# SimeonZhang/detectron2_tensorflow

Measured on AMD Instinct MI355X. Metric: img/sec whole-node Mask R-CNN R50-FPN @1333x800, higher is better.
Workload: dtype f32

## Files before the change

detectron2_tensorflow_amd/csrc/conv_mfma.hip:

```cpp
#include "common.h"
#include "conv_plan.h"
#include "internal.h"

#include <mutex>
#include <vector>

namespace d2mi {
namespace {

typedef float floatx16 __attribute__((ext_vector_type(16)));

constexpr int BK = kConvBK, LDSP = 36, LDSB = 32;

__device__ __forceinline__ int swz(int row, int elem) {
  return row * LDSB + ((((elem >> 3) ^ (row >> 2)) & 3) << 3) + (elem & 7);
}

typedef short bf16x8 __attribute__((ext_vector_type(8)));

enum EpiFlags {
  kRelu = 1, kReluAfterResidual = 2, kSplit3 = 4, kFlipTaps = 8, kMaskByResidual = 16
};

#ifndef D2MI_CONV_ABLATE
#define D2MI_CONV_ABLATE 0
#endif
constexpr int kAblate = D2MI_CONV_ABLATE;

constexpr bool kPrioMfma = true;

struct ConvArgs {
  const float* x;
  const float* w;
  const float* bias;
  const float* topdown;
  const float* residual;
  const float* gate;
  float* y;
  float* partial;
  int N, H, W, Cin, Cout, KH, KW, stride, pad, OH, OW, flags;
  int M, nM, nN, ntiles, splits, kt_per_split, nk, cchunks;
  int tile_base, m_base, m_end;
  int lds_epi;
  int nt_store;
  int x_bytes, w_bytes;
  int tdH, tdW;
  int reg_partials;
  int xcd2;
  int nlev;
  const float* lv_x[kMaxConvLevels];
  float* lv_y[kMaxConvLevels];
  const float* lv_gate[kMaxConvLevels];
  int lv_H[kMaxConvLevels], lv_W[kMaxConvLevels], lv_OH[kMaxConvLevels], lv_OW[kMaxConvLevels];
  int lv_N[kMaxConvLevels], lv_xbytes[kMaxConvLevels], lv_tile0[kMaxConvLevels + 1];
  int lv_moff[kMaxConvLevels + 1];
  const int32_t* rows;
  const int32_t* nrows;
  int rows_stride;
};

struct Geo {
  const float* x;
  float* y;
  const float* gate;
  int N, H, W, OH, OW, M, m_end, x_bytes;
  int pstride, prow0;
};

__device__ __forceinline__ Geo geo_of(const ConvArgs& a) {
  return Geo{a.x, a.y, a.gate, a.N, a.H, a.W, a.OH, a.OW, a.M, a.m_end, a.x_bytes,
             a.m_end - a.m_base, a.m_base};
}

__device__ __forceinline__ Geo select_level(const ConvArgs& a, int& tile) {
  Geo r = geo_of(a);
  if (a.nlev == 0) return r;
  int base = 0;
#pragma unroll
  for (int l = 0; l < kMaxConvLevels; ++l) {
    if (l < a.nlev && tile >= a.lv_tile0[l]) {
      base = a.lv_tile0[l];
      r.x = a.lv_x[l];
      r.y = a.lv_y[l];
      r.gate = a.lv_gate[l];
      r.N = a.lv_N[l];
      r.H = a.lv_H[l];
      r.W = a.lv_W[l];
      r.OH = a.lv_OH[l];
      r.OW = a.lv_OW[l];
      r.x_bytes = a.lv_xbytes[l];
      r.prow0 = -a.lv_moff[l];
    }
  }
  tile -= base;
  r.M = r.N * r.OH * r.OW;
  r.m_end = r.M;
  r.pstride = a.lv_moff[a.nlev > 0 ? kMaxConvLevels : 0];
  return r;
}

__device__ __forceinline__ float4 ld4(const float* p) { return *reinterpret_cast<const float4*>(p); }
// ... 829 lines not shown
#pragma unroll
      for (int j = 0; j < TN; ++j)
        fb[pb][j] = *reinterpret_cast<const bf16x8*>(
            &B16[pb * BN * LDSB + swz((wc * TN + j) * 32 + li, ks * 16 + lh * 8)]);
    };
    auto mm1 = [&](int pa, int pb) {
      if constexpr ((kAblate & 4) != 0) {
        asm volatile("" ::"v"(fa[pa][0]), "v"(fa[pa][1]), "v"(fb[pb][0]), "v"(fb[pb][1]));
        return;
      }
#pragma unroll
      for (int i = 0; i < TM; ++i)
#pragma unroll
        for (int j = 0; j < TN; ++j)
          acc[i][j] =
              __builtin_amdgcn_mfma_f32_32x32x16_bf16(fa[pa][i], fb[pb][j], acc[i][j], 0, 0, 0);
    };
    auto step16 = [&](int buf, int ks) {
      const uint16_t* A16 = reinterpret_cast<const uint16_t*>(smem + buf * STAGE);
      const uint16_t* B16 = A16 + 3 * BM * LDSB;
      ld1(A16, B16, 1, 1, ks);
      __builtin_amdgcn_sched_barrier(0);
      ld1(A16, B16, 2, 0, ks);
      mm1(1, 1);
      __builtin_amdgcn_sched_barrier(0);
      ld1(A16, B16, 0, 2, ks);
      mm1(2, 0);
      __builtin_amdgcn_sched_barrier(0);
      mm1(0, 2);
      mm1(0, 1);
      mm1(1, 0);
      mm1(0, 0);
    };
    __syncthreads();
    for (int u = 0; u < nks; ++u) {
      const int buf = u & 1;
      if (kPrioMfma) __builtin_amdgcn_s_setprio(1);
      step16(buf, 0);
      step16(buf, 1);
      if (kPrioMfma) __builtin_amdgcn_s_setprio(0);
      __builtin_amdgcn_sched_barrier(0);
      __syncthreads();
    }
  }
  if constexpr ((kAblate & 8) != 0) return;
  if (a.splits > 1 && a.reg_partials) {
    if (wave < 8) store_partial<WN, TM, TN>(a, g, acc, m0, n0, wr, wc, lane, split);
    return;
  }
  store_outputs_lds<WM, WN, TM, TN, 1024>(a, g, acc, m0, n0, wr, wc, lane, split, a.splits > 1,
                                          smem);
}

__global__ void split3_kernel(const float4* __restrict__ x, int64_t n4, uint2* __restrict__ out) {
  for (int64_t i = blockIdx.x * (int64_t)blockDim.x + threadIdx.x; i < n4;
       i += (int64_t)gridDim.x * blockDim.x) {
    uint2 h, m, l;
    split3(x[i], h, m, l);
    out[i] = h;
    out[n4 + i] = m;
    out[2 * n4 + i] = l;
  }
}

__global__ void splitk_reduce_kernel(ConvArgs a) {
  const Geo g = geo_of(a);
  const int64_t total = (int64_t)(a.m_end - a.m_base) * a.Cout;
  for (int64_t i = blockIdx.x * (int64_t)blockDim.x + threadIdx.x; i < total;
       i += (int64_t)gridDim.x * blockDim.x) {
    float acc = 0.f;
#pragma unroll 4
    for (int s = 0; s < a.splits; ++s) acc += a.partial[(size_t)s * total + i];
    const int ml = (int)(i / a.Cout), co = (int)(i - (int64_t)ml * a.Cout);
    const int m = a.m_base + ml;
    a.y[(size_t)m * a.Cout + co] = epilogue(a, g, acc, m, co);
  }
}

__device__ __forceinline__ float4 epilogue4(const ConvArgs& a, const Geo& g, float4 acc, int m,
                                            int co) {
  float4 v = acc;
  if (a.bias) {
    const float4 b = *reinterpret_cast<const float4*>(a.bias + co);
    v = make_float4(v.x + b.x, v.y + b.y, v.z + b.z, v.w + b.w);
  } else {
    v = make_float4(v.x + 0.f, v.y + 0.f, v.z + 0.f, v.w + 0.f);
  }
  const bool relu = (a.flags & kRelu) != 0, after = (a.flags & kReluAfterResidual) != 0;
  if (relu && !after) v = make_float4(fmaxf(v.x, 0.f), fmaxf(v.y, 0.f), fmaxf(v.z, 0.f), fmaxf(v.w, 0.f));
  if (a.topdown) {
    const int n = m / (g.OH * g.OW);
    const int rem = m - n * g.OH * g.OW;
    const int oh = rem / g.OW, ow = rem - oh * g.OW;
    const float4 t = *reinterpret_cast<const float4*>(
        a.topdown + (((size_t)n * a.tdH + (oh >> 1)) * a.tdW + (ow >> 1)) * a.Cout + co);
    v = make_float4(v.x + t.x, v.y + t.y, v.z + t.z, v.w + t.w);
  }
  if (a.residual) {
    const float4 r = *reinterpret_cast<const float4*>(a.residual + (size_t)m * a.Cout + co);
    v = make_float4(v.x + r.x, v.y + r.y, v.z + r.z, v.w + r.w);
  }
  if (relu && after) v = make_float4(fmaxf(v.x, 0.f), fmaxf(v.y, 0.f), fmaxf(v.z, 0.f), fmaxf(v.w, 0.f));
  if (g.gate) {
    const float4 q = *reinterpret_cast<const float4*>(g.gate + (size_t)m * a.Cout + co);
    if (!(q.x > 0.f)) v.x = 0.f;
    if (!(q.y > 0.f)) v.y = 0.f;
// ... 209 lines not shown
  D2MI_REQUIRE(n >= 0 && (n == 0 || (w_hwio && dims && w_packed)), "bad pack table");
  PackMany p = {};
  auto flush = [&]() -> int {
    if (p.n == 0) return 0;
    hipLaunchKernelGGL(pack_weights_many_kernel, dim3(p.block0[p.n]), dim3(256), 0,
                       as_stream(stream), p);
    D2MI_LAUNCH_CHECK();
    p = PackMany{};
    return 0;
  };
  for (int i = 0; i < n; ++i) {
    const int KH = dims[4 * i], KW = dims[4 * i + 1], Cin = dims[4 * i + 2], Cout = dims[4 * i + 3];
    D2MI_REQUIRE(KH > 0 && KW > 0 && Cin > 0 && Cout > 0, "bad conv weight shape (entry %d)", i);
    if (Cin % 64 != 0) {
      const int rc = d2mi_conv_pack_weights(w_hwio[i], KH, KW, Cin, Cout, w_packed[i], stream);
      if (rc) return rc;
      continue;
    }
    const long long blocks = (long long)KH * KW * ((Cout + 63) / 64) * (Cin / 64);
    if (p.n == kMaxPack || (long long)p.block0[p.n] + blocks > (1LL << 30)) {
      const int rc = flush();
      if (rc) return rc;
    }
    p.w[p.n] = w_hwio[i];
    p.out[p.n] = w_packed[i];
    p.Cin[p.n] = Cin;
    p.Cout[p.n] = Cout;
    p.block0[p.n + 1] = p.block0[p.n] + (int)blocks;
    ++p.n;
  }
  return flush();
}

extern "C" int d2mi_conv_pack_weights(const float* w_hwio, int KH, int KW, int Cin, int Cout,
                                      float* w_packed, void* stream) {
  D2MI_REQUIRE(KH > 0 && KW > 0 && Cin > 0 && Cout > 0, "bad conv weight shape");
  if (Cin % 64 == 0) {
    hipLaunchKernelGGL(pack_weights_tiled_kernel, dim3((Cout + 63) / 64, Cin / 64, KH * KW),
                       dim3(256), 0, as_stream(stream), w_hwio, Cin, Cout, w_packed);
    D2MI_LAUNCH_CHECK();
    return 0;
  }
  const int64_t total = (int64_t)KH * KW * Cin * Cout;
  const int grid = (int)std::min<int64_t>((total + 255) / 256, 8192);
  hipLaunchKernelGGL(pack_weights_kernel, dim3(grid), dim3(256), 0, as_stream(stream), w_hwio,
                     KH * KW, Cin, Cout, w_packed);
  D2MI_LAUNCH_CHECK();
  return 0;
}

template <bool SPLIT, bool ML>
static void launch_conv(int family, dim3 grid, hipStream_t st, const ConvArgs& a) {
  if (family == kConvWS256x128) {
    if constexpr (SPLIT && !ML) hipLaunchKernelGGL((conv_ws_kernel<2>), grid, dim3(1024), 0, st, a);
  } else if (family == kConv128x128) {
    hipLaunchKernelGGL((conv_mfma_kernel<2, 2, 2, 2, false, SPLIT, 3, ML>), grid, dim3(256), 0, st,
                       a);
  } else if (family == kConv128x64) {
    hipLaunchKernelGGL((conv_mfma_kernel<4, 1, 1, 2, true, SPLIT, 2, ML>), grid, dim3(256), 0, st,
                       a);
  } else {
    hipLaunchKernelGGL((conv_mfma_kernel<4, 1, 1, 1, true, SPLIT, 2, ML>), grid, dim3(256), 0, st,
                       a);
  }
}

template <int TN, int KMAX>
static void launch_stream1x1_t(const ConvPlan& p, hipStream_t st, const ConvArgs& a) {
  const int nt = tuning(kTuneConvStreamNt);
  constexpr int W = 8;
  const dim3 grid(p.grid);
  if (p.form == 3) {
    if constexpr (TN == 2)
      hipLaunchKernelGGL((conv1x1_stream_kernel<TN, KMAX, W, true, true>), grid, dim3(64 * W), 0,
                         st, a, p.nslices, nt);
  } else if (p.form == 1) {
    hipLaunchKernelGGL((conv1x1_stream_kernel<TN, KMAX, W, true, false>), grid, dim3(64 * W), 0,
                       st, a, p.nslices, nt);
  } else if (p.form == 2) {
    hipLaunchKernelGGL((conv1x1_stream_kernel<TN, KMAX, W, false, true>), grid, dim3(64 * W), 0,
                       st, a, p.nslices, nt);
  } else {
    hipLaunchKernelGGL((conv1x1_stream_kernel<TN, KMAX, W, false, false>), grid, dim3(64 * W), 0,
                       st, a, p.nslices, nt);
  }
}

static void launch_stream1x1(const ConvPlan& p, hipStream_t st, const ConvArgs& a) {
  if (p.kmax == 64 && p.tn == 4)
    launch_stream1x1_t<4, 64>(p, st, a);
  else if (p.kmax == 64)
    launch_stream1x1_t<2, 64>(p, st, a);
  else if (p.kmax == 128 && p.tn == 4)
    launch_stream1x1_t<4, 128>(p, st, a);
  else if (p.kmax == 128)
    launch_stream1x1_t<2, 128>(p, st, a);
  else
    launch_stream1x1_t<2, 256>(p, st, a);
}

static int conv_check_shape(int N, int H, int W, int Cin, int Cout, int KH, int KW, int stride) {
  D2MI_REQUIRE(N > 0 && H > 0 && W > 0 && Cin > 0 && Cout > 0 && KH > 0 && KW > 0 && stride > 0,
               "bad conv shape");
  D2MI_REQUIRE(Cin % 4 == 0, "Cin must be a multiple of 4 (got %d)", Cin);
  D2MI_REQUIRE((int64_t)H * W * Cin * sizeof(float) < (1ll << 31),
               "one conv input image must be < 2 GiB");
  D2MI_REQUIRE((int64_t)KH * KW * Cin * Cout * sizeof(float) < (1ll << 31),
               "conv weights must be < 2 GiB");
  return 0;
}
static int conv_chunk(int N, int H, int W, int Cin) {
  const int64_t img_bytes = (int64_t)H * W * Cin * sizeof(float);
  return N * img_bytes >= (1ll << 31) ? (int)(((1ll << 31) - 1) / img_bytes) : N;
}

extern "C" size_t d2mi_conv2d_workspace_size(int N, int H, int W, int Cin, int Cout, int KH,
                                             int KW, int stride, int pad_beg, int pad_end) {
  ConvPlan p;
  if (plan_conv({N, H, W, Cin, Cout, KH, KW, stride, pad_beg, pad_end}, kSplit3,
                kOpAllAligned | kOpWorkspace, SIZE_MAX, device_cus(), &p))
    return 0;
  return p.ws_bytes;
}

extern "C" int d2mi_conv2d_plan(int N, int H, int W, int Cin, int Cout, int KH, int KW, int stride,
                                int pad_beg, int pad_end, int flags, int operands,
                                size_t workspace_bytes, int32_t* out, int out_len) {
  D2MI_REQUIRE((flags & ~31) == 0 && (operands & ~127) == 0, "conv plan: unknown flag or operand bits");
  if (conv_check_shape(N, H, W, Cin, Cout, KH, KW, stride)) return -1;
  if (flags & kMaskByResidual)
    operands = (operands & ~(kOpResidual | kOpGate)) | (operands & kOpResidual ? kOpGate : 0);
  ConvPlan p;
  D2MI_REQUIRE(plan_conv({std::min(N, conv_chunk(N, H, W, Cin)), H, W, Cin, Cout, KH, KW, stride,
                          pad_beg, pad_end},
                         flags, operands, workspace_bytes, device_cus(), &p) == 0,
               "conv output is empty");
  const ConvLaunch &m = p.main, &t = p.tail;
  const int32_t v[] = {p.family, p.occ, p.split3, p.lds_epi, p.M, p.BM, p.BN, p.nM, p.nN, p.nk,
                       m.tile0, m.tiles, m.splits, m.kt_per_split, m.m_base, m.m_end, m.reduce,
                       m.reduce_grid, t.tile0, t.tiles, t.splits, t.kt_per_split, t.m_base, t.m_end,
                       t.reduce, t.reduce_grid, p.kmax, p.tn, p.form, p.nslices, p.grid,
                       (int32_t)(p.ws_bytes & 0x7fffffff), (int32_t)(p.ws_bytes >> 31)};
  return emit_plan(v, (int)(sizeof(v) / sizeof(v[0])), out, out_len);
}

struct RowList {
  const int32_t* rows;
  const int32_t* nrows;
  int cap;
};

static int conv_core(const float* x, const float* w_packed, const float* bias,
                     const float* topdown, const float* residual, const float* gate, float* y,
                     int N, int H, int W, int Cin, int Cout, int KH, int KW, int stride,
                     int pad_beg, int pad_end, int flags, void* workspace,
                     size_t workspace_bytes, void* stream, const RowList* rl = nullptr) {
  ConvPlan p;
  D2MI_REQUIRE(plan_conv({N, H, W, Cin, Cout, KH, KW, stride, pad_beg, pad_end}, flags,
                         plan_operands(topdown, residual, gate, y, bias, workspace),
                         workspace_bytes, device_cus(), &p) == 0,
               "conv output is empty");
  ConvSpace sp;
  Workspace carve(workspace, workspace_bytes);
  sp.lay(carve, p, Cout);
  ConvArgs a = {};
  a.x = x;
  a.x_bytes = (int)((int64_t)N * H * W * Cin * 4);
  a.w_bytes = (int)((int64_t)KH * KW * Cin * Cout * 4);
  a.w = w_packed;
  a.bias = bias;
  a.topdown = topdown;
  a.residual = residual;
  a.gate = gate;
  a.y = y;
  a.N = N;
  a.H = H;
  a.W = W;
  a.Cin = Cin;
  a.Cout = Cout;
  a.KH = KH;
  a.KW = KW;
  a.stride = stride;
  a.pad = pad_beg;
  a.OH = p.OH;
  a.OW = p.OW;
  a.flags = flags;
  a.M = p.M;
  a.lds_epi = p.lds_epi;
  a.reg_partials = tuning(kTuneConvEpi) != 0;
  a.xcd2 = tuning(kTuneConvXCD) != 0;
  a.nt_store = tuning(kTuneConvNt) != 0;
  a.nM = p.nM;
  a.nN = p.nN;
  a.nk = p.nk;
  a.cchunks = (Cin + BK - 1) / BK;
  a.tdH = (a.OH + 1) / 2;
  a.tdW = (a.OW + 1) / 2;
  a.ntiles = p.main.tiles;
  a.m_end = p.main.m_end;
  a.splits = p.main.splits;
  a.kt_per_split = p.main.kt_per_split;
  hipStream_t st = as_stream(stream);
  if (p.family == kConvStream1x1) {
    launch_stream1x1(p, st, a);
    D2MI_LAUNCH_CHECK();
    return 0;
  }
  auto launch = [&](const ConvLaunch& l, float* slab) {
    if (l.tiles == 0) return 0;
    ConvArgs c = a;
    c.tile_base = l.tile0;
    c.ntiles = l.tiles;
    c.m_base = l.m_base;
    c.m_end = l.m_end;
    c.splits = l.splits;
    c.kt_per_split = l.kt_per_split;
    c.partial = l.splits > 1 ? slab : nullptr;
    const dim3 g(l.tiles, l.splits);
    if (p.split3)
      launch_conv<true, false>(p.family, g, st, c);
    else
      launch_conv<false, false>(p.family, g, st, c);
    D2MI_LAUNCH_CHECK();
    if (l.reduce == kReduceNone) return 0;
    if (l.reduce == kReduceFloat4)
      hipLaunchKernelGGL(splitk_reduce4_kernel, dim3(l.reduce_grid), dim3(256), 0, st, c);
    else
      hipLaunchKernelGGL(splitk_reduce_kernel, dim3(l.reduce_grid), dim3(256), 0, st, c);
    D2MI_LAUNCH_CHECK();
    return 0;
  };
  if (rl != nullptr) {
    const ConvLaunch& l = p.main;
    ConvArgs c = a;
    c.m_base = 0;
    c.m_end = l.m_end;
    const int C4 = Cout / 4;
    hipLaunchKernelGGL(rows_fill_kernel,
                       dim3((unsigned)std::min<int64_t>(((int64_t)l.m_end * C4 + 255) / 256, 8192)),
                       dim3(256), 0, st, c);
    D2MI_LAUNCH_CHECK();
    c.rows = rl->rows;
    c.nrows = rl->nrows;
// ... 275 lines not shown
```

detectron2_tensorflow_amd/csrc/conv_plan.h:

```cpp
#pragma once
#include <stdint.h>

#include <algorithm>

#include "tuning.h"
#include "workspace.h"

namespace d2mi {

constexpr int kConvBK = 32;
constexpr int kWgradKP = 32;
constexpr int kMaxConvLevels = 6;
constexpr int kPlanSplit3 = 4;
constexpr int kPlanAccum = 8;

enum PlanOperands {
  kOpTopdown = 1,
  kOpResidual = 2,
  kOpGate = 4,
  kOpAligned = 8,
  kOpBiasAligned = 16,
  kOpWorkspace = 32,
  kOpWsAligned = 64,
  kOpAllAligned = kOpAligned | kOpBiasAligned | kOpWsAligned,
};

inline int conv_dims(int H, int W, int KH, int KW, int stride, int pb, int pe, int& OH, int& OW) {
  OH = (H + pb + pe - KH) / stride + 1;
  OW = (W + pb + pe - KW) / stride + 1;
  return (OH > 0 && OW > 0) ? 0 : -1;
}

struct StepSplit {
  int splits, per;
};
inline StepSplit split_steps(int n, int want) {
  const int per = (n + want - 1) / want;
  return {(n + per - 1) / per, per};
}

inline StepSplit conv_split_k(int ntiles, int nk, int slots) {
  int want = 1;
  if (4 * ntiles < 3 * slots && nk >= 16)
    want = std::min(std::max(1, slots / std::max(ntiles, 1)), std::min(nk / 8, 16));
  return split_steps(nk, want);
}

enum ConvFamily {
  kConv128x128 = 0,
  kConv128x64 = 1,
  kConv128x32 = 2,
  kConvWS256x128 = 3,
  kConvStream1x1 = 4,
};
enum PlanReduce { kReduceNone = 0, kReduceScalar = 1, kReduceFloat4 = 2 };

inline int conv_occ(int family) {
  if (family >= kConvWS256x128) return 1;
  return family == kConv128x128 ? 3 : 2;
}

inline int conv_family(int Cout, int KH, int KW, int Cin, bool wide_ok, bool split) {
  const int f = Cout <= 32 ? kConv128x32 : (Cout <= 64 || !wide_ok ? kConv128x64 : kConv128x128);
  if (f == kConv128x128 && split &&
      KH * KW * ((Cin + kConvBK - 1) / kConvBK) >= tuning(kTuneConvWSMinK) &&
      KH * KW <= 32)
    return kConvWS256x128;
  return f;
}
inline int conv_bm(int family) { return family == kConvWS256x128 ? 256 : 128; }
inline int conv_bn(int family) {
  return family == kConv128x64 ? 64 : family == kConv128x32 ? 32 : 128;
}

struct ConvLaunch {
  int tile0, tiles, splits, kt_per_split, m_base, m_end, reduce, reduce_grid;
};

struct ConvPlan {
  int family, occ, split3, lds_epi;
  int M, OH, OW, BM, BN, nM, nN, nk;
  ConvLaunch main, tail;
  int kmax, tn, form, nslices, grid;
  size_t ws_bytes;
};

struct ConvSpace {
  float *main, *tail;
  template <typename A>
  void lay(A& a, const ConvPlan& p, int Cout) {
    main = tail = nullptr;
    if (p.main.splits > 1)
      main = a.template take<float>((size_t)p.main.splits * (p.main.m_end - p.main.m_base) * Cout);
    if (p.tail.tiles > 0)
      tail = a.template take<float>((size_t)p.tail.splits * (p.tail.m_end - p.tail.m_base) * Cout);
  }
};

struct ConvShape {
  int N, H, W, Cin, Cout, KH, KW, stride, pad_beg, pad_end;
};

inline int plan_conv(const ConvShape& s, int flags, int operands, size_t workspace_bytes, int cus,
                     ConvPlan* out) {
  ConvPlan p = {};
  int OH, OW;
  if (conv_dims(s.H, s.W, s.KH, s.KW, s.stride, s.pad_beg, s.pad_end, OH, OW)) return -1;
  const int M = s.N * OH * OW, Cout = s.Cout, Cin = s.Cin;
  const bool split = (flags & kPlanSplit3) != 0, one_by_one = s.KH == 1 && s.KW == 1;
  const bool aligned = (operands & kOpAligned) != 0;
  p.M = M;
  p.OH = OH;
  p.OW = OW;
  p.split3 = split;
  p.lds_epi = Cout % 4 == 0 && aligned && (operands & kOpWsAligned) != 0;
  p.family = conv_family(Cout, s.KH, s.KW, Cin, p.lds_epi != 0, split);
  p.occ = conv_occ(p.family);
  p.BM = conv_bm(p.family);
  p.BN = conv_bn(p.family);
  p.nM = (M + p.BM - 1) / p.BM;
  p.nN = (Cout + p.BN - 1) / p.BN;
  p.nk = s.KH * s.KW * ((Cin + kConvBK - 1) / kConvBK);
  const int ntiles = p.nM * p.nN;
  const int G = p.occ * cus;
  const bool stream256 = one_by_one && Cin == 256 && M >= 32768 && (Cout <= 64 || Cout == 512) &&
                         Cout % 4 == 0;
  const int gs = tuning(kTuneConvSplitSlots) > 0 ? tuning(kTuneConvSplitSlots)
                                                 : (p.family == kConvWS256x128 ? 1 : 2) * cus;
  const StepSplit ks = conv_split_k(ntiles, p.nk, gs);
  p.main = {0, ntiles, ks.splits, ks.per, 0, M, kReduceNone, 0};
  p.tail = {ntiles, 0, 1, p.nk, M, M, kReduceNone, 0};
  if (ks.splits == 1 && ntiles > G && p.nk >= std::max(2, tuning(kTuneConvTailMinK)) &&
      tuning(kTuneConvTail) != 0 && !stream256) {
    const int full = (ntiles / G) * G / p.nN * p.nN;
    const int tail = ntiles - full;
    const int want = tail > 0 && 2 * tail <= G ? std::min(std::min(G / tail, p.nk / 4), 32) : 1;
    if (want >= 2) {
      const StepSplit ts = split_steps(p.nk, want);
      p.main.tiles = full;
      p.tail = {full, tail, ts.splits, ts.per, full / p.nN * p.BM, M, kReduceNone, 0};
    }
  }
  p.ws_bytes = layout_bytes<ConvSpace>(p, Cout);
  if (p.ws_bytes > workspace_bytes || !(operands & kOpWorkspace)) {
    p.main = {0, ntiles, 1, p.nk, 0, M, kReduceNone, 0};
    p.tail = {ntiles, 0, 1, p.nk, M, M, kReduceNone, 0};
    p.ws_bytes = 0;
  }
  const bool bias_al = (operands & kOpBiasAligned) != 0, ws_al = (operands & kOpWsAligned) != 0;
  const bool wide = Cout % 4 == 0 && ws_al && aligned && bias_al;
  for (ConvLaunch* l : {&p.main, &p.tail}) {
    if (l->tiles == 0 || l->splits == 1) continue;
    const int64_t total = (int64_t)(l->m_end - l->m_base) * Cout;
    l->reduce = wide ? kReduceFloat4 : kReduceScalar;
    l->reduce_grid = wide ? (int)std::min<int64_t>((total / 4 + 255) / 256, 8192)
                          : (int)std::min<int64_t>((total + 255) / 256, 4096);
  }
  const int tv = tuning(kTuneConvStream);
  const bool res = (operands & kOpResidual) != 0, gate = (operands & kOpGate) != 0;
  if (tv != 0 && split && one_by_one && s.stride == 1 && s.pad_beg == 0 &&
      !(operands & kOpTopdown) && (Cin == 64 || Cin == 128 || Cin == 256) &&
      M >= (tv < 0 ? -tv : tv) && Cout % 4 == 0 && aligned && bias_al &&
      !(Cin == 256 && ((res && gate) || !(tv < 0 || stream256)))) {
    p.family = kConvStream1x1;
    p.occ = conv_occ(p.family);
    p.kmax = Cin;
    p.form = (res ? 1 : 0) | (gate ? 2 : 0);
    const int nstrips = (M + 31) / 32;
    const bool few = (long long)nstrips * ((Cout + 127) / 128) < 8LL * cus;
    p.tn = (Cin == 256 || (res && gate) || few) ? 2 : 4;
    p.nslices = (Cout + 32 * p.tn - 1) / (32 * p.tn);
    int groups = std::max(1, cus / p.nslices / 8);
    groups = std::min(groups, std::max(1, nstrips / 8 / 8));
    p.grid = 8 * groups * p.nslices;
  }
// ... 163 lines not shown
```

detectron2_tensorflow_amd/csrc/tuning.h:

```cpp
#pragma once

namespace d2mi {

#define D2MI_TUNE_KNOBS(X)                       \
  X(kTuneConvEpi, "conv_epi", 1)                 \
  X(kTuneWgradWS1, "wgrad_ws1", 6)               \
  X(kTuneWgradXCD, "wgrad_xcd", 1)               \
  X(kTuneConvXCD, "conv_xcd", 1)                 \
  X(kTuneConvWSMinK, "conv_ws_mink", 16)         \
  X(kTuneRoiPixGrid, "roi_pix_grid", 8192)       \
  X(kTuneConvStream, "conv_stream", 8192)        \
  X(kTuneRetinaFused, "retina_fused", 1)         \
  X(kTuneRpnMerge, "rpn_merge", 1)               \
  X(kTuneNmsScan, "nms_scan", 1)                 \
  X(kTuneRoiHeavy, "roi_heavy", 16)              \
  X(kTuneRpnCompact, "rpn_compact", 1)           \
  X(kTuneConvStreamNt, "conv_stream_nt", 2)      \
  X(kTuneConvNt, "conv_nt", 0)                   \
  X(kTuneConvTailMinK, "conv_tail_mink", 8)      \
  X(kTuneSgdRev, "sgd_rev", 0)                   \
  X(kTuneRetinaRank, "retina_rank", 0)           \
  X(kTuneSoloMfma, "solo_mfma", 2)               \
  X(kTuneRetinaVar, "retina_var", 12018)         \
  X(kTuneConvSplitSlots, "conv_split_slots", 0)  \
  X(kTuneConvTail, "conv_tail", 1)               \
  X(kTuneWgradOcc3MinP, "wgrad_occ3_min_p", 65536) \
  X(kTuneWgradSlots, "wgrad_slots", 0)           \
  X(kTuneWgradMinCh, "wgrad_minch", 16)          \
  X(kTuneWgradMaxSplit, "wgrad_maxsplit", 128)   \
  X(kTuneWgradPrio, "wgrad_prio", 1)             \
  X(kTuneTopkFloor, "topk_floor", 1)
enum TuneKey {
#define X(id, key, def) id,
  D2MI_TUNE_KNOBS(X)
#undef X
  kTuneCount
};
int tuning(TuneKey k);

}
```

detectron2_tensorflow_amd/layers/ops.py:

```python
import math
import os

import numpy as np
import torch

from .. import _C
from ..utils import capture, host_sync
from . import handoff

_DEFAULT_SCALE_CLAMP = math.log(1000.0 / 16)

BOX_MODE_RAW, BOX_MODE_ALIGNED, BOX_MODE_UNALIGNED = 0, 1, 2


class KernelTimer:

    enabled = False
    detail = False
    records = []

    @classmethod
    def reset(cls, enabled=True, detail=False):
        cls.enabled = enabled
        cls.detail = detail
# ... 764 lines not shown
            raise ValueError("accumulate_into must be the (dw, db) of a wgrad of this shape")
    else:
        dw = torch.empty((KH, KW, Cin, Cout), dtype=torch.float32, device=x.device)
        db = torch.empty((Cout,), dtype=torch.float32, device=x.device) if with_bias else None
    args = (N, H, W, Cin, Cout, KH, KW, int(stride), int(pb), int(pe))
    wsb = _WGRAD_WS.get(args)
    if wsb is None:
        wsb = _WGRAD_WS[args] = _C.lib().d2mi_conv2d_wgrad_workspace_size(*args)
    if accumulate_into is not None:
        wsb = max(wsb, (KH * KW * Cin * Cout + Cout) * 4)
    ws = _C.scratch(wsb, x.device) if wsb else None
    ev = KernelTimer.start()
    flags = (4 if math_mode == "split" else 0) | (8 if accumulate_into is not None else 0)
    if census is not None:
        rc = _C.lib().d2mi_conv2d_wgrad_rows(_C.ptr(x), _C.ptr(dy), _C.ptr(dw), _C.ptr(db), *args,
                                             flags, _C.ptr(census.ws), census.ws.numel(),
                                             _C.ptr(ws), wsb, _C.stream_of(x.device))
        if rc == 1:
            KernelTimer.stop(ev, "conv2d_wgrad_rows", 0.0)
            if KernelTimer.detail and ev is not None:
                KernelTimer.stop(ev, f"wgrad_rows {N}x{H}x{W}x{Cin}->{Cout} k{KH} s{stride}", 0.0)
            census.used()
            return (dw, db) if with_bias else dw
        rc = min(rc, 0)
    else:
        rc = _C.lib().d2mi_conv2d_wgrad_ex(_C.ptr(x), _C.ptr(dy), _C.ptr(dw), _C.ptr(db), *args,
                                           flags, _C.ptr(ws), wsb, _C.stream_of(x.device))
    fl = 2.0 * dy.numel() * KH * KW * Cin
    group = "conv2d_wgrad_split" if flags & 4 else "conv2d_wgrad_mfma"
    KernelTimer.stop(ev, group, fl)
    if ev is not None:
        byts = 4.0 * (x.numel() + dy.numel() + dw.numel() * (2 if accumulate_into is not None else 1)
                      + (Cout if with_bias else 0))
        KernelTimer.stop(ev, f"{group}_{bound_of(fl, byts, math_mode)}_bound", fl,
                         extra=lambda: {"bytes": byts})
    if KernelTimer.detail and ev is not None:
        KernelTimer.stop(ev, f"wgrad {N}x{H}x{W}x{Cin}->{Cout} k{KH} s{stride}", fl,
                         extra=lambda: {"bytes": byts})
    _C.check(rc, "d2mi_conv2d_wgrad")
    return (dw, db) if with_bias else dw


OP_TOPDOWN, OP_RESIDUAL, OP_GATE, OP_ALIGNED, OP_BIAS_ALIGNED, OP_WORKSPACE, OP_WS_ALIGNED = (
    1, 2, 4, 8, 16, 32, 64)
OP_ALL_ALIGNED = OP_ALIGNED | OP_BIAS_ALIGNED | OP_WS_ALIGNED
CONV_FAMILIES = ("tiled128x128", "tiled128x64", "tiled128x32", "ws256x128", "stream1x1")
WGRAD_KERNELS = ("f32", "split", "split_occ3", "ws", "ws_inc")
_LAUNCH_FIELDS = ("tile0", "tiles", "splits", "kt_per_split", "m_base", "m_end", "reduce",
                  "reduce_grid")
CONV_PLAN_FIELDS = (("family", "occ", "split3", "lds_epi", "M", "BM", "BN", "nM", "nN", "nk")
                    + tuple("main_" + f for f in _LAUNCH_FIELDS)
                    + tuple("tail_" + f for f in _LAUNCH_FIELDS)
                    + ("stream_kmax", "stream_tn", "stream_form", "stream_nslices", "stream_grid"))
LEVELS_PLAN_FIELDS = ("family", "occ", "split3", "lds_epi", "BM", "BN", "nN", "nk", "tiles",
                      "splits", "kt_per_split", "reduce_grid", "nlev")
WGRAD_PLAN_FIELDS = ("kernel", "TM", "TN", "BM", "BN", "nCi", "nCo", "tiles", "nchunks", "splits",
                     "chunks_per_split", "part", "reduce", "reduce_grid")


def _plan_query(fn, name, args, flags, operands, workspace_bytes, n):
    out = (_C.ctypes.c_int32 * n)()
    rc = fn(*args, int(flags), int(operands), int(workspace_bytes), out, n)
    _C.check(min(rc, 0), name)
    v = list(out)
    return v[:-2], v[-2] | (v[-1] << 31)


def conv_plan(N, H, W, Cin, Cout, k, stride=1, pad=(0, 0), flags=4,
              operands=OP_ALL_ALIGNED | OP_WORKSPACE, workspace_bytes=None):
    args = (N, H, W, Cin, Cout, k, k, int(stride), int(pad[0]), int(pad[1]))
    lib = _C.lib()
    if workspace_bytes is None:
        workspace_bytes = lib.d2mi_conv2d_workspace_size(*args)
    v, wsb = _plan_query(lib.d2mi_conv2d_plan, "d2mi_conv2d_plan", args, flags, operands,
                         workspace_bytes, len(CONV_PLAN_FIELDS) + 2)
    return dict(zip(CONV_PLAN_FIELDS, v), workspace_bytes=wsb)


def conv_levels_plan(dims, Cin, Cout, k, stride=1, pad=(0, 0), flags=4,
                     operands=OP_ALL_ALIGNED | OP_WORKSPACE, workspace_bytes=None):
    dm = _C.host_array(_C.ctypes.c_int32, [int(d) for lv in dims for d in lv])
    args = (dm, len(dims), Cin, Cout, k, k, int(stride), int(pad[0]), int(pad[1]))
    lib = _C.lib()
    if workspace_bytes is None:
        workspace_bytes = lib.d2mi_conv2d_levels_workspace_size(*args)
    v, wsb = _plan_query(lib.d2mi_conv2d_levels_plan, "d2mi_conv2d_levels_plan", args, flags,
                         operands, workspace_bytes, len(LEVELS_PLAN_FIELDS) + 16)
    n = len(LEVELS_PLAN_FIELDS)
    return dict(zip(LEVELS_PLAN_FIELDS, v), tile0=v[n:n + 7], moff=v[n + 7:n + 14],
                workspace_bytes=wsb)


def wgrad_plan(N, H, W, Cin, Cout, k, stride=1, pad=(0, 0), flags=4,
               operands=OP_ALL_ALIGNED | OP_WORKSPACE, workspace_bytes=None):
    args = (N, H, W, Cin, Cout, k, k, int(stride), int(pad[0]), int(pad[1]))
    lib = _C.lib()
    if workspace_bytes is None:
        workspace_bytes = lib.d2mi_conv2d_wgrad_workspace_size(*args)
    v, wsb = _plan_query(lib.d2mi_conv2d_wgrad_plan, "d2mi_conv2d_wgrad_plan", args, flags,
                         operands, workspace_bytes, len(WGRAD_PLAN_FIELDS) + 2)
    return dict(zip(WGRAD_PLAN_FIELDS, v), workspace_bytes=wsb)


class _FoldFrozenBNFn(torch.autograd.Function):

    @staticmethod
    def forward(ctx, w, bias, gamma, beta, mean, var, eps, want_packed):
        _C.require_device(w, mean, var)
        KH, KW, Cin, Cout = w.shape
        w = _f32c(w)
        w_eff = torch.empty_like(w)
        packed = (torch.empty((KH, KW, Cout, Cin), dtype=torch.float32, device=w.device)
                  if want_packed else None)
        b_eff = torch.empty((Cout,), dtype=torch.float32, device=w.device)
        rc = _C.lib().d2mi_fold_frozen_bn(_C.ptr(w), _C.ptr(bias), _C.ptr(gamma), _C.ptr(beta),
                                          _C.ptr(mean), _C.ptr(var), float(eps), KH, KW, Cin,
                                          Cout, _C.ptr(w_eff), _C.ptr(packed), _C.ptr(b_eff),
                                          _C.stream_of(w.device))
        _C.check(rc, "d2mi_fold_frozen_bn")
        ctx.save_for_backward(w, bias, gamma, mean, var)
        ctx.set_materialize_grads(False)
        ctx.eps = float(eps)
        ctx.has = (bias is not None, gamma is not None, beta is not None)
        if packed is not None:
            ctx.mark_non_differentiable(packed)
        return w_eff, b_eff, packed

    @staticmethod
    def backward(ctx, gw_eff, gb_eff, _gpacked):
# ... 1398 lines not shown
```

Baseline: 113.9.

## Add KW-sharing warp-specialized conv kernel reusing input strip across horizontal taps

Adds a warp-specialized 256x128 conv kernel for stride-1 2- or 3-wide filters. Producer waves load one contiguous input row strip into LDS per kernel row, and the MFMA waves reuse it for every horizontal tap by shifting the row offset, instead of reloading and re-splitting the A tile per tap. This is meant to cut global loads and split3 conversion work for 3x3 convs. The cost is a larger LDS footprint and more complex indexing. It is gated by a planner condition, tuning knobs (on by default) and a minimum tile count, and the plan query is extended to report strip fields.

```diff
diff --git a/detectron2_tensorflow_amd/csrc/conv_mfma.hip b/detectron2_tensorflow_amd/csrc/conv_mfma.hip
--- a/detectron2_tensorflow_amd/csrc/conv_mfma.hip
+++ b/detectron2_tensorflow_amd/csrc/conv_mfma.hip
@@ -47,6 +47,7 @@
   int tdH, tdW;
   int reg_partials;
   int xcd2;
+  int kw_share;
   int nlev;
   const float* lv_x[kMaxConvLevels];
   float* lv_y[kMaxConvLevels];
@@ -982,6 +983,268 @@
                                           smem);
 }
 
+template <int KW>
+__global__ __launch_bounds__(1024, 1) void conv_ws_kw_kernel(ConvArgs a) {
+  constexpr int WM = 4, WN = 2, TM = 2, TN = 2;
+  constexpr int BM = 256, BN = 128, RB = 2;
+  constexpr int SR = kStripRowsMax;
+  constexpr int NSLOT = (SR + 63) / 64;
+  constexpr int SA = (NSLOT + KW - 1) / KW;
+  constexpr int PAD = (KW - 1) / 2;
+  constexpr int A_ELEMS = 3 * SR * LDSB, B_ELEMS = 3 * BN * LDSB;
+  static_assert(BM + KW - 1 <= SR && NSLOT * 64 >= SR && (A_ELEMS * 2) % 16 == 0, "strip layout");
+  static_assert(2 * (A_ELEMS + B_ELEMS) * 2 <= kLdsBytes, "LDS budget");
+  __shared__ __attribute__((aligned(16))) float smem[A_ELEMS + B_ELEMS];
+  static_assert(A_ELEMS + B_ELEMS >= 32 * (BN + 4), "LDS epilogue slab does not fit");
+  uint16_t* const smem16 = reinterpret_cast<uint16_t*>(smem);
+
+  const int tid = threadIdx.x;
+  const int lane = tid & 63;
+  const int wave = __builtin_amdgcn_readfirstlane(tid >> 6);
+  const int wr = wave / WN, wc = wave % WN;
+
+  int split;
+  const int tile = a.tile_base + xcd_tile(a.xcd2, split);
+  const int kt0 = split * a.kt_per_split;
+  const int kt1 = min(a.nk, kt0 + a.kt_per_split);
+  const int nks = max(kt1 - kt0, 0);
+  const Geo g = geo_of(a);
+  const int mt = tile / a.nN, nt = tile - mt * a.nN;
+  const int m0 = mt * BM, n0 = nt * BN;
+  const int R0 = m0 / g.OW, ow0 = m0 - R0 * g.OW;
+  const int G0 = kt0 / KW;
+
+  floatx16 acc[TM][TN];
+  if (wave >= 8) {
+    const int st = tid - 512;
+    const int srow = st >> 3, schunk = (st & 7) * 4;
+    int base[NSLOT];
+    uint32_t hv[NSLOT];
+#pragma unroll
+    for (int p = 0; p < NSLOT; ++p) {
+      const int q = srow + 64 * p;
+      const int e = q + ow0 + 1 - PAD;
+      const int j = e / (g.W + 1);
+      const int xs = e - j * (g.W + 1) - 1;
+      const int R = R0 + j;
+      const int n = R / g.OH, oh = R - n * g.OH;
+      const bool ok = xs >= 0 && R < g.N * g.OH && q < SR;
+      const int ihv = oh - a.pad;
+      base[p] = ((n * g.H + ihv) * g.W + xs) * a.Cin + schunk;
+      uint32_t b = 0;
+      for (int kh = 0; kh < a.KH; ++kh)
+        b |= (ok && (unsigned)(ihv + kh) < (unsigned)g.H) ? 1u << kh : 0u;
+      hv[p] = b;
+    }
+    const __amdgpu_buffer_rsrc_t xrsrc = __builtin_amdgcn_make_buffer_rsrc(
+        const_cast<float*>(g.x), 0, g.x_bytes, 0x00020000);
+    const __amdgpu_buffer_rsrc_t wrsrc = __builtin_amdgcn_make_buffer_rsrc(
+        const_cast<float*>(a.w), 0, a.w_bytes, 0x00020000);
+    constexpr uint32_t kOOB = 0x80000000u;
+    const int taps = a.KH * KW;
+    int boff[RB];
+    bool bco[RB];
+#pragma unroll
+    for (int p = 0; p < RB; ++p) {
+      const int co = n0 + srow + 64 * p;
+      bco[p] = co < a.Cout;
+      boff[p] = co * a.Cin + schunk;
+    }
+    const int klast = kt0 + max(nks, 1) - 1;
+    int l_s = G0 * KW, l_chunk = G0 / a.KH, l_kh = G0 - (G0 / a.KH) * a.KH;
+    int b_kt = kt0, b_chunk = kt0 / taps, b_tap = kt0 - (kt0 / taps) * taps;
+    auto load = [&](int kw, float4 (&la)[SA], float4 (&lb)[RB]) {
+      if constexpr ((kAblate & 1) != 0) return;
+      {
+        const int cc = b_chunk * BK;
+        const bool cok = cc + schunk < a.Cin;
+        const int wtap = (a.flags & kFlipTaps) ? taps - 1 - b_tap : b_tap;
+        const int wsc = wtap * a.Cout * a.Cin + cc;
+#pragma unroll
+        for (int p = 0; p < RB; ++p) {
+          const uint32_t off = (cok & bco[p]) ? (uint32_t)(boff[p] + wsc) * 4u : kOOB;
+          lb[p] = __builtin_bit_cast(float4, __builtin_amdgcn_raw_buffer_load_b128(wrsrc, off, 0, 0));
+        }
+      }
+      const int cc = l_chunk * BK;
+      const bool cok = cc + schunk < a.Cin;
+      const int toff = l_kh * g.W * a.Cin + cc;
+#pragma unroll
+      for (int i = 0; i < SA; ++i) {
+        const int p = kw * SA + i;
+        if (p >= NSLOT) continue;
+        const bool inb = ((hv[p] >> l_kh) & 1u) != 0;
+        const uint32_t off = (cok & inb) ? (uint32_t)(base[p] + toff) * 4u : kOOB;
+        la[i] = __builtin_bit_cast(float4, __builtin_amdgcn_raw_buffer_load_b128(xrsrc, off, 0, 0));
+      }
+      ++l_s;
+      if (kw == KW - 1 && ++l_kh == a.KH) {
+        l_kh = 0;
+        ++l_chunk;
+      }
+      if (l_s - KW + 1 > b_kt && b_kt < klast) {
+        ++b_kt;
+        if (++b_tap == taps) {
+          b_tap = 0;
+          ++b_chunk;
+        }
+      }
+    };
+    auto write_b = [&](int s, const float4 (&lb)[RB]) {
+      if constexpr ((kAblate & 2) != 0) {
+#pragma unroll
+        for (int p = 0; p < RB; ++p) asm volatile("" ::"v"(lb[p].x));
+        return;
+      }
+      const int bk = min(max(s - KW + 1, kt0), klast) - kt0;
+      uint16_t* B16 = smem16 + 2 * A_ELEMS + (bk & 1) * B_ELEMS;
+#pragma unroll
+      for (int p = 0; p < RB; ++p) {
+        uint2 h, m, l;
+        split3(lb[p], h, m, l);
+        const int o = swz(srow + 64 * p, schunk);
+        *reinterpret_cast<uint2*>(&B16[o]) = h;
+        *reinterpret_cast<uint2*>(&B16[BN * LDSB + o]) = m;
+        *reinterpret_cast<uint2*>(&B16[2 * BN * LDSB + o]) = l;
+      }
+    };
+    auto write_a = [&](int s, int kw, const float4 (&la)[SA]) {
+      if constexpr ((kAblate & 2) != 0) {
+#pragma unroll
+        for (int i = 0; i < SA; ++i)
+          if (kw * SA + i < NSLOT) asm volatile("" ::"v"(la[i].x));
+        return;
+      }
+      uint16_t* A16 = smem16 + ((s / KW - G0) & 1) * A_ELEMS;
+#pragma unroll
+      for (int i = 0; i < SA; ++i) {
+        const int p = kw * SA + i;
+        if (p >= NSLOT) continue;
+        uint2 h, m, l;
+        split3(la[i], h, m, l);
+        const int q = srow + 64 * p;
+        const int o = swz(q, schunk);
+        if (64 * p + 63 < SR || q < SR) {
+          *reinterpret_cast<uint2*>(&A16[o]) = h;
+          *reinterpret_cast<uint2*>(&A16[SR * LDSB + o]) = m;
+          *reinterpret_cast<uint2*>(&A16[2 * SR * LDSB + o]) = l;
+        }
+      }
+    };
+    if (nks == 0) {
+      __syncthreads();
+    } else {
+      float4 ra[KW][SA], rb[KW][RB];
+      if constexpr ((kAblate & 1) != 0) {
+#pragma unroll
+        for (int j = 0; j < KW; ++j) {
+#pragma unroll
+          for (int p = 0; p < SA; ++p) ra[j][p] = make_float4(1.f, 2.f, 3.f, 4.f);
+#pragma unroll
+          for (int p = 0; p < RB; ++p) rb[j][p] = make_float4(1.f, 2.f, 3.f, 4.f);
+        }
+      }
+#pragma unroll
+      for (int kw = 0; kw < KW; ++kw) load(kw, ra[kw], rb[kw]);
+      const int sbar = kt0 - 1 + KW, slast = kt1 - 1 + KW;
+      const int send = ((kt1 - 1) / KW + 1) * KW;
+      int s = G0 * KW;
+      for (; s < send; s += KW) {
+#pragma unroll
+        for (int kw = 0; kw < KW; ++kw) {
+          write_a(s + kw, kw, ra[kw]);
+          write_b(s + kw, rb[kw]);
+          load(kw, ra[kw], rb[kw]);
+          if (s + kw >= sbar) __syncthreads();
+        }
+      }
+#pragma unroll
+      for (int kw = 0; kw < KW; ++kw) {
+        if (s + kw <= slast) {
+          if (s + kw < slast) write_b(s + kw, rb[kw]);
+          if (s + kw >= sbar) __syncthreads();
+        }
+      }
+    }
+  } else {
+#pragma unroll
+    for (int i = 0; i < TM; ++i)
+#pragma unroll
+      for (int j = 0; j < TN; ++j)
+#pragma unroll
+        for (int r = 0; r < 16; ++r) acc[i][j][r] = 0.f;
+    const int li = lane & 31, lh = lane >> 5;
+    int pos[TM];
+#pragma unroll
+    for (int i = 0; i < TM; ++i) {
+      const int r = (wr * TM + i) * 32 + li;
+      pos[i] = r + (ow0 + r) / g.OW;
+    }
+    bf16x8 fa[3][TM], fb[3][TN];
+    int ao[TM];
+    auto ld1 = [&](const uint16_t* A16, const uint16_t* B16, int pa, int pb, int ks) {
+#pragma unroll
+      for (int i = 0; i < TM; ++i)
+        fa[pa][i] = *reinterpret_cast<const bf16x8*>(&A16[pa * SR * LDSB + (ao[i] ^ (ks * 16))]);
+#pragma unroll
+      for (int j = 0; j < TN; ++j)
+        fb[pb][j] = *reinterpret_cast<const bf16x8*>(
+            &B16[pb * BN * LDSB + swz((wc * TN + j) * 32 + li, ks * 16 + lh * 8)]);
+    };
+    auto mm1 = [&](int pa, int pb) {
+      if constexpr ((kAblate & 4) != 0) {
+        asm volatile("" ::"v"(fa[pa][0]), "v"(fa[pa][1]), "v"(fb[pb][0]), "v"(fb[pb][1]));
+        return;
+      }
+#pragma unroll
+      for (int i = 0; i < TM; ++i)
+#pragma unroll
+        for (int j = 0; j < TN; ++j)
+          acc[i][j] =
+              __builtin_amdgcn_mfma_f32_32x32x16_bf16(fa[pa][i], fb[pb][j], acc[i][j], 0, 0, 0);
+    };
+    auto step16 = [&](const uint16_t* A16, const uint16_t* B16, int ks) {
+      ld1(A16, B16, 1, 1, ks);
+      __builtin_amdgcn_sched_barrier(0);
+      ld1(A16, B16, 2, 0, ks);
+      mm1(1, 1);
+      __builtin_amdgcn_sched_barrier(0);
+      ld1(A16, B16, 0, 2, ks);
+      mm1(2, 0);
+      __builtin_amdgcn_sched_barrier(0);
+      mm1(0, 2);
+      mm1(0, 1);
+      mm1(1, 0);
+      mm1(0, 0);
+    };
+    int c_kw = kt0 - G0 * KW, sbuf = 0;
+    __syncthreads();
+    for (int u = 0; u < nks; ++u) {
+      const uint16_t* A16 = smem16 + sbuf * A_ELEMS;
+      const uint16_t* B16 = smem16 + 2 * A_ELEMS + (u & 1) * B_ELEMS;
+#pragma unroll
+      for (int i = 0; i < TM; ++i) ao[i] = swz(pos[i] + c_kw, lh * 8);
+      if (kPrioMfma) __builtin_amdgcn_s_setprio(1);
+      step16(A16, B16, 0);
+      step16(A16, B16, 1);
+      if (kPrioMfma) __builtin_amdgcn_s_setprio(0);
+      if (++c_kw == KW) {
+        c_kw = 0;
+        sbuf ^= 1;
+      }
+      __builtin_amdgcn_sched_barrier(0);
+      __syncthreads();
+    }
+  }
+  if constexpr ((kAblate & 8) != 0) return;
+  if (a.splits > 1 && a.reg_partials) {
+    if (wave < 8) store_partial<WN, TM, TN>(a, g, acc, m0, n0, wr, wc, lane, split);
+    return;
+  }
+  store_outputs_lds<WM, WN, TM, TN, 1024>(a, g, acc, m0, n0, wr, wc, lane, split, a.splits > 1,
+                                          smem);
+}
+
 __global__ void split3_kernel(const float4* __restrict__ x, int64_t n4, uint2* __restrict__ out) {
   for (int64_t i = blockIdx.x * (int64_t)blockDim.x + threadIdx.x; i < n4;
        i += (int64_t)gridDim.x * blockDim.x) {
@@ -1297,7 +1560,14 @@
 template <bool SPLIT, bool ML>
 static void launch_conv(int family, dim3 grid, hipStream_t st, const ConvArgs& a) {
   if (family == kConvWS256x128) {
-    if constexpr (SPLIT && !ML) hipLaunchKernelGGL((conv_ws_kernel<2>), grid, dim3(1024), 0, st, a);
+    if constexpr (SPLIT && !ML) {
+      if (a.kw_share && a.KW == 3)
+        hipLaunchKernelGGL((conv_ws_kw_kernel<3>), grid, dim3(1024), 0, st, a);
+      else if (a.kw_share)
+        hipLaunchKernelGGL((conv_ws_kw_kernel<2>), grid, dim3(1024), 0, st, a);
+      else
+        hipLaunchKernelGGL((conv_ws_kernel<2>), grid, dim3(1024), 0, st, a);
+    }
   } else if (family == kConv128x128) {
     hipLaunchKernelGGL((conv_mfma_kernel<2, 2, 2, 2, false, SPLIT, 3, ML>), grid, dim3(256), 0, st,
                        a);
@@ -1371,8 +1641,10 @@
 extern "C" int d2mi_conv2d_plan(int N, int H, int W, int Cin, int Cout, int KH, int KW, int stride,
                                 int pad_beg, int pad_end, int flags, int operands,
                                 size_t workspace_bytes, int32_t* out, int out_len) {
-  D2MI_REQUIRE((flags & ~31) == 0 && (operands & ~127) == 0, "conv plan: unknown flag or operand bits");
+  D2MI_REQUIRE((flags & ~31) == 0 && (operands & ~255) == 0, "conv plan: unknown flag or operand bits");
   if (conv_check_shape(N, H, W, Cin, Cout, KH, KW, stride)) return -1;
+  const bool with_strip = (operands & kOpQueryStrip) != 0;
+  operands &= ~kOpQueryStrip;
   if (flags & kMaskByResidual)
     operands = (operands & ~(kOpResidual | kOpGate)) | (operands & kOpResidual ? kOpGate : 0);
   ConvPlan p;
@@ -1385,8 +1657,9 @@
                        m.tile0, m.tiles, m.splits, m.kt_per_split, m.m_base, m.m_end, m.reduce,
                        m.reduce_grid, t.tile0, t.tiles, t.splits, t.kt_per_split, t.m_base, t.m_end,
                        t.reduce, t.reduce_grid, p.kmax, p.tn, p.form, p.nslices, p.grid,
-                       (int32_t)(p.ws_bytes & 0x7fffffff), (int32_t)(p.ws_bytes >> 31)};
-  return emit_plan(v, (int)(sizeof(v) / sizeof(v[0])), out, out_len);
+                       (int32_t)(p.ws_bytes & 0x7fffffff), (int32_t)(p.ws_bytes >> 31),
+                       p.kw_share, p.strip_rows, p.strip_lds_bytes};
+  return emit_plan(v, (int)(sizeof(v) / sizeof(v[0])) - (with_strip ? 0 : 3), out, out_len);
 }
 
 struct RowList {
@@ -1434,6 +1707,7 @@
   a.lds_epi = p.lds_epi;
   a.reg_partials = tuning(kTuneConvEpi) != 0;
   a.xcd2 = tuning(kTuneConvXCD) != 0;
+  a.kw_share = p.kw_share;
   a.nt_store = tuning(kTuneConvNt) != 0;
   a.nM = p.nM;
   a.nN = p.nN;
diff --git a/detectron2_tensorflow_amd/csrc/conv_plan.h b/detectron2_tensorflow_amd/csrc/conv_plan.h
--- a/detectron2_tensorflow_amd/csrc/conv_plan.h
+++ b/detectron2_tensorflow_amd/csrc/conv_plan.h
@@ -23,6 +23,7 @@
   kOpWorkspace = 32,
   kOpWsAligned = 64,
   kOpAllAligned = kOpAligned | kOpBiasAligned | kOpWsAligned,
+  kOpQueryStrip = 128,
 };
 
 inline int conv_dims(int H, int W, int KH, int KW, int stride, int pb, int pe, int& OH, int& OW) {
@@ -68,6 +69,14 @@
     return kConvWS256x128;
   return f;
 }
+constexpr int kLdsBytes = 160 * 1024;
+constexpr int kStripRowBytes = 3 * 2 * kConvBK;
+constexpr int kWsBStageBytes = 128 * kStripRowBytes;
+constexpr int kStripRowsMax = (kLdsBytes - 2 * kWsBStageBytes) / (2 * kStripRowBytes);
+inline int conv_strip_rows_at(int W, int KW, int ow0) { return 256 + KW - 1 + (ow0 + 255) / W; }
+inline int conv_strip_rows(int W, int KW) { return conv_strip_rows_at(W, KW, W - 1); }
+inline int conv_strip_lds_bytes(int rows) { return 2 * rows * kStripRowBytes + 2 * kWsBStageBytes; }
+
 inline int conv_bm(int family) { return family == kConvWS256x128 ? 256 : 128; }
 inline int conv_bn(int family) {
   return family == kConv128x64 ? 64 : family == kConv128x32 ? 32 : 128;
@@ -82,6 +91,7 @@
   int M, OH, OW, BM, BN, nM, nN, nk;
   ConvLaunch main, tail;
   int kmax, tn, form, nslices, grid;
+  int kw_share, strip_rows, strip_lds_bytes;
   size_t ws_bytes;
 };
 
@@ -121,6 +131,13 @@
   p.nM = (M + p.BM - 1) / p.BM;
   p.nN = (Cout + p.BN - 1) / p.BN;
   p.nk = s.KH * s.KW * ((Cin + kConvBK - 1) / kConvBK);
+  if (p.family == kConvWS256x128 && s.stride == 1 && OW == s.W && (s.KW == 2 || s.KW == 3) &&
+      s.pad_beg == (s.KW - 1) / 2 && conv_strip_rows(s.W, s.KW) <= kStripRowsMax &&
+      tuning(kTuneConvKwShare) != 0 && p.nM * p.nN >= tuning(kTuneConvKwShareMinTiles)) {
+    p.kw_share = 1;
+    p.strip_rows = conv_strip_rows(s.W, s.KW);
+    p.strip_lds_bytes = conv_strip_lds_bytes(p.strip_rows);
+  }
   const int ntiles = p.nM * p.nN;
   const int G = p.occ * cus;
   const bool stream256 = one_by_one && Cin == 256 && M >= 32768 && (Cout <= 64 || Cout == 512) &&
diff --git a/detectron2_tensorflow_amd/csrc/tuning.h b/detectron2_tensorflow_amd/csrc/tuning.h
--- a/detectron2_tensorflow_amd/csrc/tuning.h
+++ b/detectron2_tensorflow_amd/csrc/tuning.h
@@ -29,7 +29,9 @@
   X(kTuneWgradMinCh, "wgrad_minch", 16)          \
   X(kTuneWgradMaxSplit, "wgrad_maxsplit", 128)   \
   X(kTuneWgradPrio, "wgrad_prio", 1)             \
-  X(kTuneTopkFloor, "topk_floor", 1)
+  X(kTuneTopkFloor, "topk_floor", 1)             \
+  X(kTuneConvKwShare, "conv_kw_share", 1)        \
+  X(kTuneConvKwShareMinTiles, "conv_kw_share_mintiles", 512)
 enum TuneKey {
 #define X(id, key, def) id,
   D2MI_TUNE_KNOBS(X)
diff --git a/detectron2_tensorflow_amd/layers/ops.py b/detectron2_tensorflow_amd/layers/ops.py
--- a/detectron2_tensorflow_amd/layers/ops.py
+++ b/detectron2_tensorflow_amd/layers/ops.py
@@ -840,6 +840,8 @@
                     + tuple("main_" + f for f in _LAUNCH_FIELDS)
                     + tuple("tail_" + f for f in _LAUNCH_FIELDS)
                     + ("stream_kmax", "stream_tn", "stream_form", "stream_nslices", "stream_grid"))
+CONV_STRIP_FIELDS = ("kw_share", "strip_rows", "strip_lds_bytes")
+OP_QUERY_STRIP = 128
 LEVELS_PLAN_FIELDS = ("family", "occ", "split3", "lds_epi", "BM", "BN", "nN", "nk", "tiles",
                       "splits", "kt_per_split", "reduce_grid", "nlev")
 WGRAD_PLAN_FIELDS = ("kernel", "TM", "TN", "BM", "BN", "nCi", "nCo", "tiles", "nchunks", "splits",
@@ -860,9 +862,14 @@
     lib = _C.lib()
     if workspace_bytes is None:
         workspace_bytes = lib.d2mi_conv2d_workspace_size(*args)
-    v, wsb = _plan_query(lib.d2mi_conv2d_plan, "d2mi_conv2d_plan", args, flags, operands,
-                         workspace_bytes, len(CONV_PLAN_FIELDS) + 2)
-    return dict(zip(CONV_PLAN_FIELDS, v), workspace_bytes=wsb)
+    n = len(CONV_PLAN_FIELDS) + 2
+    out = (_C.ctypes.c_int32 * (n + 3))()
+    rc = lib.d2mi_conv2d_plan(*args, int(flags), int(operands) | OP_QUERY_STRIP,
+                              int(workspace_bytes), out, n + 3)
+    _C.check(min(rc, 0), "d2mi_conv2d_plan")
+    v = list(out)
+    return dict(zip(CONV_PLAN_FIELDS, v), workspace_bytes=v[n - 2] | (v[n - 1] << 31),
+                **dict(zip(CONV_STRIP_FIELDS, v[n:])))
 
 
 def conv_levels_plan(dims, Cin, Cout, k, stride=1, pad=(0, 0), flags=4,
```

Result: no change. 113.7 (-0.2%).
